# nacho-pancho/binary-image-compression

Hardware: AMD Instinct MI355X
Metric: encode MPixels/s (and MB/s out) at 1/2/4/8 GPUs; bit-exact vs CPU (higher is better)
Workload: dtype u64; 1 GPU; c3: 16384x16384 8-bit gray -> 8 bitplanes -> med -> per-row runs -> Golomb + EG streams per plane (bitplanes formed in registers, not returned: planes NULL) -- the count pass writes the EG stream, the Golomb emission reads the residual rows from it; rows=16384, cols=16384, planes_per_gpu=8, parallelism=dp1 (independent images per GPU)

## Files before the change

### binary-image-compression_amd/csrc/bic_capi.cpp

```cpp
#include "bic_ctx.h"

#include <cctype>
#include <cmath>
#include <map>
#include <new>

#ifdef BIC_STAMPS
namespace bic {
int read_stamps(uint64_t* host, size_t n);
int read_match_stamps(uint64_t* host, size_t n);
}
#endif

namespace {

int ctx_init(bic_ctx* ctx) {
  if (hipStreamCreateWithFlags(&ctx->own, hipStreamNonBlocking) != hipSuccess) return BIC_EDEVICE;
  ctx->cur = ctx->own;
  uint64_t host_lut[bic::kLutWords];
  bic::build_byte_lut(host_lut);
  bic::egad_build_nib(host_lut + bic::kLutEgadNib);
  bic::egad_build_dec_nib(host_lut + bic::kLutEgadDec);
  if (hipMalloc(&ctx->lut, sizeof(host_lut)) != hipSuccess ||
      hipMemcpy(ctx->lut, host_lut, sizeof(host_lut), hipMemcpyHostToDevice) != hipSuccess)
// ... 219 lines not shown
    if (!pnm_int(bytes, n, i, h)) return BIC_EINVAL;
    pnm_skip_comments(bytes, n, i);
    if (!pnm_int(bytes, n, i, mv)) return BIC_EINVAL;
    if (w <= 0 || h <= 0 || mv <= 0 || mv > 65535) return BIC_EINVAL;
    ++i;
  } else {
    return BIC_EINVAL;
  }
  if (i > n) return BIC_EINVAL;
  info->type = type;
  info->cols = (size_t)w;
  info->rows = (size_t)h;
  info->maxval = (int)mv;
  info->data_offset = i;
  return BIC_OK;
}

double bic_enum_codelength(unsigned n, unsigned r) {
  if (r == 0 || r >= n) return 0.0;
  const unsigned m = r * 2 > n ? n - r : r;
  if (m == 1) {
    if ((n & (n - 1)) == 0) {
      unsigned e = 0;
      while ((1u << e) < n) ++e;
      return (double)e;
    }
    return (double)std::log2((long double)n);
  }
  const long double ln = std::lgamma((long double)n + 1.0L) - std::lgamma((long double)m + 1.0L) -
                         std::lgamma((long double)(n - m) + 1.0L);
  return (double)(ln * 1.442695040888963407359924681001892137L);
}

int bic_tile_lentab(unsigned W, uint64_t* lentab) {
  if (W < 1 || W > 64 || !lentab) return BIC_EINVAL;
  const unsigned M = W * W;
  for (unsigned w = 0; w <= M; ++w)
    lentab[w] = (uint64_t)(2.0 + bic_enum_codelength(M, w));
  return BIC_OK;
}

int bic_prof_enable(bic_ctx* ctx, int on) {
  if (!ctx) return BIC_EINVAL;
  ctx->prof_on = on != 0;
  return BIC_OK;
}

int bic_prof_only(bic_ctx* ctx, const char* name) {
  if (!ctx) return BIC_EINVAL;
  ctx->prof_only = name ? name : "";
  return BIC_OK;
}

int bic_prof_collect(bic_ctx* ctx, char* buf, size_t cap) {
  int rc = bind(ctx);
  if (rc) return rc;
  if (!buf || cap == 0) return BIC_EINVAL;
  BIC_HIP(hipStreamSynchronize(ctx->cur));
  std::map<std::string, std::pair<unsigned long, double>> agg;
  for (auto& r : ctx->recs) {
    float ms = 0.f;
    if (hipEventElapsedTime(&ms, r.a, r.b) != hipSuccess) ms = -1.f;
    auto& e = agg[r.name];
    e.first += 1;
    e.second += ms;
    ctx->pool.push_back(r.a);
    ctx->pool.push_back(r.b);
  }
  ctx->recs.clear();
  (void)hipGetLastError();
  std::string outs;
  for (auto& kv : agg) {
    char line[160];
    std::snprintf(line, sizeof line, "%s %lu %.6f\n", kv.first.c_str(), kv.second.first, kv.second.second);
    outs += line;
  }
  std::snprintf(buf, cap, "%s", outs.c_str());
  return outs.size() < cap ? BIC_OK : BIC_ENOSPC;
}

#ifdef BIC_STAMPS
int bic_debug_stamps(uint64_t* host, size_t n) { return bic::read_stamps(host, n); }
int bic_debug_match_stamps(uint64_t* host, size_t n) { return bic::read_match_stamps(host, n); }
#endif

}
```

### binary-image-compression_amd/csrc/bic_kernels.hip

```cpp
#include "bic_device.h"
#include "bic_k1pi.h"
#include "bic_kstat.h"

namespace bic {

__device__ __forceinline__ uint64_t transpose8x8(uint64_t x) {
  uint64_t t;
  t = (x ^ (x >> 7)) & 0x00AA00AA00AA00AAull;
  x = x ^ t ^ (t << 7);
  t = (x ^ (x >> 14)) & 0x0000CCCC0000CCCCull;
  x = x ^ t ^ (t << 14);
  t = (x ^ (x >> 28)) & 0x00000000F0F0F0F0ull;
  x = x ^ t ^ (t << 28);
  return x;
}

template <bool VEC>
__global__ __launch_bounds__(kBlock) void k_bitplanes_u8(const uint8_t* __restrict__ gray, size_t pitch,
                                                         uint32_t rows, uint32_t cols, uint32_t used,
                                                         int plane0, int nplanes, uint64_t* __restrict__ planes,
                                                         uint32_t wpr) {
  const uint32_t groups = (used + 63) / 64;
  const uint64_t gw = (uint64_t)blockIdx.x * kWaves + wave_id();
  if (gw >= (uint64_t)rows * groups) return;
// ... 427 lines not shown
    LaneK k;
    uint64_t D[LW], R[LW];
#pragma unroll
    for (int i = 0; i < LW; ++i) D[i] = PREDICT ? cur[i] ^ up[i] : cur[i];
    const uint64_t dl = wave_shr1_u64(D[LW - 1]);
#pragma unroll
    for (int i = 0; i < LW; ++i) {
      const uint32_t w = w0 + i;
      R[i] = D[i];
      if constexpr (PREDICT) {
        R[i] = D[i] ^ ((D[i] >> 1) | ((i ? D[i - 1] : dl) << 63));
        if (row == 0 && w == 0) R[i] &= ~BIC_MSB;
      }
      R[i] = w < g.used ? (w == g.used - 1 ? R[i] & g.trail : R[i]) : 0;
      lanek_word(k, R[i], (int32_t)(w * 64));
      up[i] = cur[i];
    }
    const uint64_t id = (uint64_t)plane * g.rows + row;
    lanek_store(k, krec + id, kpos + id, sones + id);
    uint64_t* orow = out + (uint64_t)row * g.wpr;
#pragma unroll
    for (int i = 0; i < LW; i += 2)
      if (w0 + i < g.wpr)
        *reinterpret_cast<ulonglong2*>(orow + w0 + i) =
            store_r ? make_ulonglong2(R[i], R[i + 1]) : make_ulonglong2(cur[i], cur[i + 1]);
    for (uint32_t w = 64 * LW + 2 * lane; w < g.wpr; w += 128)
      *reinterpret_cast<ulonglong2*>(orow + w) = make_ulonglong2(0, 0);
#pragma unroll
    for (int i = 0; i < LW; ++i) cur[i] = nxt[i];
  }
}

void launch_pbm_rows(hipStream_t s, const uint8_t* raster, uint64_t stride, const Geom& g, int predict, uint64_t* dst,
                     bool store_resid, uint32_t* sones, int4* krec, uint32_t* kpos, uint32_t* zero) {
  constexpr int RPW = 8;
  const uint32_t wpp = (g.rows + RPW - 1) / RPW;
  const uint32_t grid = (uint32_t)(((uint64_t)wpp * g.nplanes + kWaves - 1) / kWaves);
  const int sr = store_resid && predict ? 1 : 0;
#define BIC_PKS(LW, P) k_pbm_kstat<LW, RPW, P><<<grid, kBlock, 0, s>>>(g, raster, stride, dst, sr, sones, krec, kpos, zero)
  if (g.used <= 128) { if (predict) BIC_PKS(2, true); else BIC_PKS(2, false); }
  else { if (predict) BIC_PKS(4, true); else BIC_PKS(4, false); }
#undef BIC_PKS
}

#ifndef BIC_GRAY_ROWS
#define BIC_GRAY_ROWS 4
#endif
#ifndef BIC_GRAY_ROWS_BM
#define BIC_GRAY_ROWS_BM 1
#endif
constexpr int kGrayRowsP = BIC_GRAY_ROWS, kGrayRowsBM = BIC_GRAY_ROWS_BM;
uint32_t gray_strips(const Geom& g) { return (g.used + 63) / 64; }

__device__ __forceinline__ void perm_t4(uint32_t w0, uint32_t w1, uint32_t w2, uint32_t w3, uint32_t (&out)[4]) {
  const uint32_t a01 = __builtin_amdgcn_perm(w0, w1, 0x04000501u), b01 = __builtin_amdgcn_perm(w0, w1, 0x06020703u);
  const uint32_t a23 = __builtin_amdgcn_perm(w2, w3, 0x04000501u), b23 = __builtin_amdgcn_perm(w2, w3, 0x06020703u);
  out[0] = __builtin_amdgcn_perm(a01, a23, 0x07060302u);
  out[1] = __builtin_amdgcn_perm(a01, a23, 0x05040100u);
  out[2] = __builtin_amdgcn_perm(b01, b23, 0x07060302u);
  out[3] = __builtin_amdgcn_perm(b01, b23, 0x05040100u);
}

__device__ __forceinline__ uint64_t transpose8x8_bs(uint32_t x0, uint32_t x1) {
  uint32_t hi = __builtin_bswap32(x0), lo = __builtin_bswap32(x1);
  uint32_t t;
  t = __builtin_amdgcn_bitop3_b32(lo, lo >> 7, 0x00AA00AAu, 0x28);
  lo = __builtin_amdgcn_bitop3_b32(lo, t, t << 7, 0x96);
  t = __builtin_amdgcn_bitop3_b32(hi, hi >> 7, 0x00AA00AAu, 0x28);
  hi = __builtin_amdgcn_bitop3_b32(hi, t, t << 7, 0x96);
  t = __builtin_amdgcn_bitop3_b32(lo, lo >> 14, 0x0000CCCCu, 0x28);
  lo = __builtin_amdgcn_bitop3_b32(lo, t, t << 14, 0x96);
  t = __builtin_amdgcn_bitop3_b32(hi, hi >> 14, 0x0000CCCCu, 0x28);
  hi = __builtin_amdgcn_bitop3_b32(hi, t, t << 14, 0x96);
  t = __builtin_amdgcn_bitop3_b32(lo, hi << 4, 0xF0F0F0F0u, 0x28);
  lo ^= t;
  hi ^= t >> 4;
  return ((uint64_t)hi << 32) | lo;
}

template <bool FULL = false>
__device__ __forceinline__ void gray_to_planes(const uint4 (&v)[4], uint64_t (&pw)[8], uint64_t mask) {
  uint64_t T[8];
#pragma unroll
  for (int i = 0; i < 4; ++i) {
    T[2 * i] = transpose8x8_bs(v[i].x, v[i].y);
    T[2 * i + 1] = transpose8x8_bs(v[i].z, v[i].w);
  }
  uint32_t XL[4], YL[4], XH[4], YH[4];
  perm_t4((uint32_t)T[0], (uint32_t)T[1], (uint32_t)T[2], (uint32_t)T[3], XL);
  perm_t4((uint32_t)T[4], (uint32_t)T[5], (uint32_t)T[6], (uint32_t)T[7], YL);
  perm_t4((uint32_t)(T[0] >> 32), (uint32_t)(T[1] >> 32), (uint32_t)(T[2] >> 32), (uint32_t)(T[3] >> 32), XH);
  perm_t4((uint32_t)(T[4] >> 32), (uint32_t)(T[5] >> 32), (uint32_t)(T[6] >> 32), (uint32_t)(T[7] >> 32), YH);
#pragma unroll
  for (int b = 0; b < 4; ++b) {
    pw[b] = ((uint64_t)XL[b] << 32) | YL[b];
    pw[4 + b] = ((uint64_t)XH[b] << 32) | YH[b];
    if constexpr (!FULL) {
      pw[b] &= mask;
      pw[4 + b] &= mask;
    }
  }
}

#ifndef BIC_GRAY_PREFETCH
#define BIC_GRAY_PREFETCH 1
#endif
constexpr bool kGrayPrefetch = BIC_GRAY_PREFETCH != 0;
#ifndef BIC_GRAY_BYTEMED
#define BIC_GRAY_BYTEMED 1
#endif
constexpr bool kGrayByteMed = BIC_GRAY_BYTEMED != 0;
template <bool PREDICT, bool STORE_R>
constexpr int gray_rows_per_wave() { return kGrayByteMed && PREDICT && STORE_R ? kGrayRowsBM : kGrayRowsP; }
__device__ __forceinline__ void load64_mis(const uint8_t* src, uint4 (&v)[4]) {
  const uintptr_t a = reinterpret_cast<uintptr_t>(src);
  const uint32_t mis = (uint32_t)(a & 15), bs = mis & 3, dq = mis >> 2;
  const uint4* b = reinterpret_cast<const uint4*>(src - mis);
  uint32_t in[20];
#pragma unroll
  for (int q = 0; q < 4; ++q) {
    const uint4 x = b[q];
    in[4 * q] = x.x;
    in[4 * q + 1] = x.y;
    in[4 * q + 2] = x.z;
    in[4 * q + 3] = x.w;
  }
  const uint4 x4 = mis ? b[4] : make_uint4(0, 0, 0, 0);
  in[16] = x4.x;
  in[17] = x4.y;
  in[18] = x4.z;
  in[19] = x4.w;
#define BIC_MIS_CASE(DQ)                                                                                    \
  case DQ:                                                                                                  \
    _Pragma("unroll") for (int q = 0; q < 4; ++q) v[q] =                                                    \
        make_uint4(__builtin_amdgcn_alignbyte(in[4 * q + DQ + 1], in[4 * q + DQ], bs),                     \
                   __builtin_amdgcn_alignbyte(in[4 * q + DQ + 2], in[4 * q + DQ + 1], bs),                 \
                   __builtin_amdgcn_alignbyte(in[4 * q + DQ + 3], in[4 * q + DQ + 2], bs),                 \
                   __builtin_amdgcn_alignbyte(in[4 * q + DQ + 4], in[4 * q + DQ + 3], bs));                \
    break;
  switch (dq) {
    BIC_MIS_CASE(0)
    BIC_MIS_CASE(1)
    BIC_MIS_CASE(2)
    default: BIC_MIS_CASE(3)
  }
#undef BIC_MIS_CASE
}

struct Raw16 {
  uint4 cur[8], up[8];
};

template <bool PREDICT, bool FULL, bool STORE_R, bool NP8, bool EGS, bool MIS = false, int S16 = 0>
// ... 1420 lines not shown
```

### binary-image-compression_amd/csrc/bic_kstat.h

```cpp
#pragma once
#include "bic_device.h"

namespace bic {

constexpr int32_t kNoOnes = 1 << 30;
constexpr uint32_t kMaxStrips = 4;

__device__ __forceinline__ uint32_t parity_changes(uint64_t x) {
  constexpr uint64_t kEven = 0xAAAAAAAAAAAAAAAAull;
  const uint64_t E = x & kEven, O = x & ~kEven;
  const uint64_t pe = (~x + (E << 1)) & x, po = (~x + (O << 1)) & x;
  return (uint32_t)__popcll(pe & O) + (uint32_t)__popcll(po & E);
}

struct LaneK {
  uint32_t ones = 0, chg = 0;
  int32_t q0 = -kNoOnes, qh = -kNoOnes, ql = kNoOnes, first = -1, last = -1;
};
__device__ __forceinline__ void lanek_word(LaneK& k, uint64_t x, int32_t c0) {
  if (!x) return;
  const int32_t m = __popcll(x), o = (int32_t)k.ones;
  const int32_t pl = c0 + 63 - __builtin_ctzll(x), pf = c0 + __builtin_clzll(x);
  k.q0 = max(k.q0, pl - m - 2 * o);
  k.qh = max(k.qh, pl - m - 3 * o - 1);
  k.ql = min(k.ql, pf - 2 * o - m);
  k.chg += parity_changes(x) + (k.last >= 0 ? (uint32_t)((k.last ^ pf) & 1) : 0u);
  if (k.first < 0) k.first = pf;
  k.last = pl;
  k.ones += m;
}

__device__ __forceinline__ void lanek_store(const LaneK& k, int4* rec, uint32_t* pos, uint32_t* sones) {
  if (__ballot(k.ones != 0) == ~0ull) {
    const int32_t before = dpp_or<0x138>(-1, k.last);
    const uint32_t chg = k.chg + (before >= 0 ? (uint32_t)((before ^ k.first) & 1) : 0u);
    const uint32_t inc = wave_incl_sum_u32(k.ones | (chg << 16));
    const int32_t base = (int32_t)((inc & 0xffffu) - k.ones);
    const int32_t q0 = wave_max(k.q0 - 2 * base);
    const int32_t qh = wave_max(k.qh - 3 * base);
    const int32_t ql = wave_min(k.ql - 2 * base);
    const uint32_t t = lane63_u32(inc), tot = t & 0xffffu;
    const uint32_t f = (uint32_t)__builtin_amdgcn_readlane(k.first, 0);
    const uint32_t last = lane63_u32((uint32_t)k.last);
    if (lane_id() == 0) {
      *rec = make_int4(q0, qh, ql, (int32_t)(tot | (t >> 16 << 16)));
      *pos = (f & 0xffffu) | (last << 16);
      *sones = tot;
    }
    return;
  }
  const uint32_t inc = wave_incl_sum_u32(k.ones);
  const int32_t base = (int32_t)(inc - k.ones);
  const int mx = wave_incl_max(k.last);
  const int32_t before = dpp_or<0x138>(-1, mx);
  uint32_t chg = k.chg;
  int32_t first = -1;
  if (k.ones) {
    if (before >= 0) chg += (uint32_t)((before ^ k.first) & 1);
    else first = k.first;
  }
  const int32_t q0 = wave_max(k.ones ? k.q0 - 2 * base : -kNoOnes);
  const int32_t qh = wave_max(k.ones ? k.qh - 3 * base : -kNoOnes);
  const int32_t ql = wave_min(k.ones ? k.ql - 2 * base : kNoOnes);
  const uint32_t c = wave_sum_u32(chg);
  const int32_t f = wave_max(first);
  const uint32_t tot = lane63_u32(inc);
  const uint32_t last = lane63_u32((uint32_t)mx);
  if (lane_id() == 0) {
    *rec = make_int4(q0, qh, ql, (int32_t)(tot | (c << 16)));
    *pos = ((uint32_t)f & 0xffffu) | (last << 16);
    *sones = tot;
  }
}

__device__ __forceinline__ void strip_word_put(uint32_t* t, int b, uint64_t x, int32_t c0) {
  const int lane = lane_id();
  const uint32_t m = (uint32_t)__popcll(x) | (parity_changes(x) << 8);
  uint32_t hh, hl, lh, ll;
  const uint32_t xh = (uint32_t)(x >> 32), xl = (uint32_t)x;
  asm volatile("v_ffbh_u32 %0, %1" : "=v"(hh) : "v"(xh));
  asm volatile("v_ffbh_u32 %0, %1" : "=v"(hl) : "v"(xl));
  asm volatile("v_ffbl_b32 %0, %1" : "=v"(lh) : "v"(xh));
  asm volatile("v_ffbl_b32 %0, %1" : "=v"(ll) : "v"(xl));
  const uint32_t lz = min(hh, hl + 32u), tz = min(ll, lh + 32u);
  const uint32_t c = ((uint32_t)c0 + lz) | (((uint32_t)c0 + 63u - tz) << 16);
  const uint32_t idx = ((uint32_t)(lane & 7) >> 2) * 256 + 32 * b + 4 * (lane >> 3) + (lane & 3);
  t[idx] = m;
  t[512 + idx] = c;
}
template <int CTRL>
__device__ __forceinline__ int dpp_same(int v) {
  return __builtin_amdgcn_mov_dpp(v, CTRL, 0xf, 0xf, true);
}
__device__ __forceinline__ void strip_records(const uint32_t* t, int np, int4* krec, uint32_t* kpos, uint32_t* sones,
                                              uint64_t id0, uint64_t pstride) {
  const int L = lane_id(), p = L >> 3, j = L & 7;
  const uint4 a0 = *reinterpret_cast<const uint4*>(t + 4 * L);
  const uint4 a1 = *reinterpret_cast<const uint4*>(t + 256 + 4 * L);
  const uint4 c0 = *reinterpret_cast<const uint4*>(t + 512 + 4 * L);
  const uint4 c1 = *reinterpret_cast<const uint4*>(t + 768 + 4 * L);
  const uint32_t av[8] = {a0.x, a0.y, a0.z, a0.w, a1.x, a1.y, a1.z, a1.w};
  const uint32_t cv[8] = {c0.x, c0.y, c0.z, c0.w, c1.x, c1.y, c1.z, c1.w};
  uint32_t ones = 0, chg = 0;
  int32_t first = -1, last = -1, q0 = -kNoOnes, qh = -kNoOnes, ql = kNoOnes;
#pragma unroll
  for (int i = 0; i < 8; ++i) {
    const int32_t m = (int32_t)(av[i] & 0xffu);
    if (m) {
      const int32_t pf = (int32_t)(cv[i] & 0xffffu), pl = (int32_t)(cv[i] >> 16), o = (int32_t)ones;
      chg += (av[i] >> 8) + (last >= 0 ? (uint32_t)((last ^ pf) & 1) : 0u);
      q0 = max(q0, pl - m - 2 * o);
      qh = max(qh, pl - m - 1 - 3 * o);
      ql = min(ql, pf - m - 2 * o);
      if (first < 0) first = pf;
      last = pl;
      ones += (uint32_t)m;
    }
  }
  uint32_t inc = ones;
  int32_t lmax = last;
#pragma unroll
  for (int d = 1; d < 8; d <<= 1) {
    const uint32_t o = d == 1 ? (uint32_t)dpp_or<0x111>(0, (int)inc) : d == 2 ? (uint32_t)dpp_or<0x112>(0, (int)inc)
                                                                             : (uint32_t)dpp_or<0x114>(0, (int)inc);
    const int32_t lm = d == 1 ? dpp_or<0x111>(-1, lmax) : d == 2 ? dpp_or<0x112>(-1, lmax) : dpp_or<0x114>(-1, lmax);
    if (j >= d) {
      inc += o;
      lmax = max(lmax, lm);
    }
  }
  const int32_t lprev = dpp_or<0x111>(-1, lmax);
  const int32_t before = j ? lprev : -1;
  const int32_t B = (int32_t)(inc - ones);
  if (ones) {
    if (before >= 0) chg += (uint32_t)((before ^ first) & 1);
    q0 -= 2 * B;
    qh -= 3 * B;
    ql -= 2 * B;
  }
  int32_t f = ones ? first : INT_MAX;
  uint32_t tot = ones;
#define BIC_RED8(CTRL)                          \
  q0 = max(q0, dpp_same<CTRL>(q0));             \
  qh = max(qh, dpp_same<CTRL>(qh));             \
  ql = min(ql, dpp_same<CTRL>(ql));             \
  f = min(f, dpp_same<CTRL>(f));                \
  last = max(last, dpp_same<CTRL>(last));       \
  chg += (uint32_t)dpp_same<CTRL>((int)chg);    \
  tot += (uint32_t)dpp_same<CTRL>((int)tot);
  BIC_RED8(0xB1)
  BIC_RED8(0x4E)
  BIC_RED8(0x141)
#undef BIC_RED8
  if (j == 0 && p < np) {
    const uint64_t id = id0 + (uint64_t)p * pstride;
    krec[id] = make_int4(q0, qh, ql, (int32_t)(tot | (chg << 16)));
    kpos[id] = ((uint32_t)(f == INT_MAX ? -1 : f) & 0xffffu) | ((uint32_t)last << 16);
    sones[id] = tot;
  }
}

struct RowK {
  int32_t q0, qh, ql;
  uint32_t ones, chg;
};
struct RowKRaw {
  int4 v[kMaxStrips];
  uint32_t pp[kMaxStrips];
};
__device__ __forceinline__ RowKRaw row_kstats_load(const int4* rec, const uint32_t* pos, uint32_t ns) {
  RowKRaw q;
#pragma unroll
  for (uint32_t s = 0; s < kMaxStrips; ++s) {
    q.v[s] = s < ns ? rec[s] : make_int4(0, 0, 0, 0);
    q.pp[s] = s < ns ? pos[s] : 0u;
  }
  return q;
}
__device__ __forceinline__ RowK row_kstats_combine(const RowKRaw& q, uint32_t cols) {
  const int4* v = q.v;
  const uint32_t* pp = q.pp;
  RowK r{0, 0, 0, 0, 0};
  int32_t last = -1;
#pragma unroll
  for (uint32_t s = 0; s < kMaxStrips; ++s) {
    const uint32_t o = (uint32_t)v[s].w & 0xffffu;
    if (!o) continue;
    r.q0 = max(r.q0, v[s].x - 2 * (int32_t)r.ones);
    r.qh = max(r.qh, v[s].y - 3 * (int32_t)r.ones);
    r.ql = min(r.ql, v[s].z - 2 * (int32_t)r.ones);
    r.chg += ((uint32_t)v[s].w >> 16) + (uint32_t)((last ^ (int32_t)(int16_t)(pp[s] & 0xffffu)) & 1);
    r.ones += o;
    last = (int16_t)(pp[s] >> 16);
  }
  r.chg += (uint32_t)((last ^ (int32_t)cols) & 1);
  return r;
}
__device__ __forceinline__ RowK row_kstats(const int4* rec, const uint32_t* pos, uint32_t ns, uint32_t cols) {
  return row_kstats_combine(row_kstats_load(rec, pos, ns), cols);
}

}
```

### binary-image-compression_amd/pybic/__init__.py

```python
import ctypes as C
import os

import numpy as np

PKG = os.path.dirname(os.path.dirname(os.path.abspath(__file__)))
LIB_PATH = os.environ.get("BIC_LIB_PATH") or os.path.join(PKG, "lib", "libbic.so")

BIC_OK, BIC_EINVAL, BIC_ENOMEM, BIC_EDEVICE, BIC_ENOSPC, BIC_ENODEV, BIC_EDATA = range(7)
CODER_GOLOMB, CODER_EG, CODER_EG_ADAPTIVE = 0, 1, 2

EXPORTS = [
    "bic_ctx_create", "bic_ctx_destroy", "bic_ctx_set_stream", "bic_ctx_get_stream", "bic_ctx_own_stream",
    "bic_sync",
    "bic_strerror", "bic_device_count", "bic_reserve", "bic_bitplanes_u8", "bic_med_residual",
    "bic_encode_planes", "bic_encode_planes2", "bic_ctx_set_option", "bic_encode_slot_words", "bic_golomb_encode_samples", "bic_patch_encode",
    "bic_pack_streams", "bic_prof_enable", "bic_prof_collect", "bic_prof_only", "bic_enum_codelength", "bic_tile_lentab",
    "bic_malloc", "bic_free", "bic_memcpy_h2d", "bic_memcpy_d2h", "bic_memset", "bic_pbm_unpack", "bic_pbm_pack",
    "bic_patch_search", "bic_match_encode", "bic_set_match_parts", "bic_encode_gray",
    "bic_bitplanes_u8_range", "bic_encode_gray_range", "bic_encode_planes_packed", "bic_encode_gray_packed",
    "bic_row_index", "bic_decode_planes", "bic_pgm_bitplanes", "bic_pnm_parse_header",
    "bic_gf2_transpose", "bic_gf2_mul", "bic_planes_to_gray", "bic_match_encode_inv", "bic_match_encode_var", "bic_egad_row_index",
    "bic_encode_gray16", "bic_encode_gray16_packed", "bic_bitplanes_u16", "bic_decode_gray",
    "bic_encode_pbm", "bic_encode_pbm_packed", "bic_decode_pbm",
    "bic_bsvd_update_coefficients", "bic_bsvd_update_dictionary", "bic_bsvd_learn",
]

GF2_AB, GF2_ATB, GF2_ABT, GF2_ATBT = 0, 1, 2, 3


class PnmInfo(C.Structure):
    _fields_ = [("type", C.c_int), ("rows", C.c_size_t), ("cols", C.c_size_t), ("maxval", C.c_int),
                ("data_offset", C.c_size_t)]


class BicError(RuntimeError):
    def __init__(self, code, what=""):
        self.code = code
        super().__init__(f"{what}: bic error {code} ({_strerror(code)})")


_lib = None


def _strerror(code):
    try:
        return load().bic_strerror(code).decode()
    except Exception:
        return "?"


def load(path=LIB_PATH):
    global _lib
    if _lib is not None:
        return _lib
    if not os.path.exists(path):
        raise OSError(f"{path} not built; run make -C binary-image-compression_amd")
    L = C.CDLL(path)
    vp, sz, u64, i32, u32 = C.c_void_p, C.c_size_t, C.c_uint64, C.c_int, C.c_uint

    def sig(name, res, args):
        f = getattr(L, name)
        f.restype, f.argtypes = res, args

    sig("bic_ctx_create", i32, [i32, C.POINTER(vp)])
    sig("bic_ctx_destroy", i32, [vp])
    sig("bic_ctx_set_stream", i32, [vp, vp])
    sig("bic_ctx_get_stream", vp, [vp])
    sig("bic_ctx_own_stream", vp, [vp])
    sig("bic_sync", i32, [vp])
    sig("bic_strerror", C.c_char_p, [i32])
    sig("bic_device_count", i32, [C.POINTER(i32)])
    sig("bic_reserve", i32, [vp, i32, sz, sz])
    sig("bic_bitplanes_u8", i32, [vp, vp, sz, sz, sz, i32, vp, sz])
    sig("bic_med_residual", i32, [vp, vp, i32, sz, sz, sz, i32, vp, vp])
    sig("bic_encode_planes", i32, [vp, vp, i32, sz, sz, sz, i32, i32, vp, sz, vp])
    sig("bic_encode_slot_words", sz, [sz, sz, i32])
    sig("bic_encode_planes2", i32, [vp, vp, i32, sz, sz, sz, i32, vp, sz, vp, vp, sz, vp])
    sig("bic_ctx_set_option", i32, [vp, i32, C.c_long])
    sig("bic_golomb_encode_samples", i32, [vp, vp, sz, u64, u64, u32, vp, sz, vp])
    sig("bic_patch_encode", i32, [vp, vp, sz, sz, sz, u32, vp, vp, vp, vp, vp, vp, vp, sz, vp])
    sig("bic_pack_streams", i32, [vp, vp, i32, sz, vp, vp, vp])
    sig("bic_prof_enable", i32, [vp, i32])
    sig("bic_prof_collect", i32, [vp, C.c_char_p, sz])
    sig("bic_prof_only", i32, [vp, C.c_char_p])
    sig("bic_enum_codelength", C.c_double, [u32, u32])
    sig("bic_tile_lentab", i32, [u32, vp])
    sig("bic_malloc", i32, [vp, sz, C.POINTER(vp)])
    sig("bic_free", i32, [vp, vp])
    sig("bic_memcpy_h2d", i32, [vp, vp, vp, sz])
    sig("bic_memcpy_d2h", i32, [vp, vp, vp, sz])
    sig("bic_memset", i32, [vp, vp, i32, sz])
    sig("bic_pbm_unpack", i32, [vp, vp, sz, sz, vp, sz])
    sig("bic_pbm_pack", i32, [vp, vp, sz, sz, sz, vp])
    sig("bic_patch_search", i32, [vp, vp, sz, sz, sz, u32, vp, vp, vp])
    sig("bic_match_encode", i32, [vp, vp, sz, sz, sz, u32, u32, u32, vp, vp, vp, vp, vp, vp, vp, vp, vp, sz, vp])
    sig("bic_set_match_parts", i32, [vp, u32])
    sig("bic_match_encode_inv", i32, [vp, vp, sz, sz, sz, u32, u32, u32, vp, vp, vp, vp, vp, vp, vp, vp, vp, vp, sz, vp])
    sig("bic_egad_row_index", i32, [vp, vp, i32, sz, sz, sz, i32, vp])
    sig("bic_match_encode_var", i32, [vp, i32, vp, sz, sz, sz, u32, u32, u32, vp, vp, vp, vp, vp, vp, vp, vp, vp, sz, vp])
    sig("bic_encode_gray", i32, [vp, vp, sz, sz, sz, i32, vp, sz, i32, vp, sz, vp, vp, sz, vp])
    sig("bic_bitplanes_u8_range", i32, [vp, vp, sz, sz, sz, i32, i32, vp, sz])
    sig("bic_encode_gray_range", i32, [vp, vp, sz, sz, sz, i32, i32, vp, sz, i32, vp, sz, vp, vp, sz, vp])
    sig("bic_encode_planes_packed", i32, [vp, vp, i32, sz, sz, sz, i32, vp, sz, vp, vp, vp, sz, vp, vp, vp])
    sig("bic_encode_gray_packed", i32, [vp, vp, sz, sz, sz, i32, i32, vp, sz, i32, vp, sz, vp, vp, vp, sz, vp, vp, vp])
    sig("bic_row_index", i32, [vp, vp, i32, sz, sz, sz, i32, vp])
    sig("bic_decode_planes", i32, [vp, i32, vp, sz, vp, vp, vp, i32, sz, sz, sz, i32, vp, vp])
    sig("bic_pgm_bitplanes", i32, [vp, vp, sz, sz, i32, i32, i32, vp, sz])
    sig("bic_pnm_parse_header", i32, [C.c_char_p, sz, C.POINTER(PnmInfo)])
    sig("bic_gf2_transpose", i32, [vp, vp, sz, sz, sz, vp, sz])
    sig("bic_gf2_mul", i32, [vp, i32, vp, sz, sz, sz, vp, sz, sz, sz, vp, sz, sz, sz])
    sig("bic_planes_to_gray", i32, [vp, vp, i32, i32, sz, sz, sz, i32, vp, sz])
    sig("bic_bitplanes_u16", i32, [vp, vp, sz, sz, sz, i32, i32, i32, vp, sz])
    sig("bic_encode_gray16", i32, [vp, vp, sz, sz, sz, i32, i32, i32, vp, sz, i32, vp, sz, vp, vp, sz, vp])
    sig("bic_encode_gray16_packed", i32, [vp, vp, sz, sz, sz, i32, i32, i32, vp, sz, i32, vp, sz, vp, vp, vp, sz, vp,
                                          vp, vp])
    sig("bic_decode_gray", i32, [vp, i32, vp, sz, vp, vp, vp, i32, i32, sz, sz, i32, vp, i32, i32, vp, sz])
    sig("bic_encode_pbm", i32, [vp, vp, sz, i32, sz, sz, vp, sz, i32, vp, sz, vp, vp, sz, vp])
    sig("bic_encode_pbm_packed", i32, [vp, vp, sz, i32, sz, sz, vp, sz, i32, vp, sz, vp, vp, vp, sz, vp, vp, vp])
    sig("bic_decode_pbm", i32, [vp, i32, vp, sz, vp, vp, vp, i32, sz, sz, i32, vp, vp, sz])
    sig("bic_bsvd_update_coefficients", i32, [vp, vp, sz, sz, sz, vp, sz, sz, vp, sz, vp])
    sig("bic_bsvd_update_dictionary", i32, [vp, vp, sz, sz, sz, vp, sz, sz, vp, sz, vp])
    sig("bic_bsvd_learn", i32, [vp, vp, sz, vp, sz, sz, sz, vp, sz, sz, vp, sz, sz, C.POINTER(sz)])
    _lib = L
    return L


def as_u64(t):
    return t.detach().cpu().numpy().view(np.uint64)


def stream_bytes(words_i64, nbits):
    nw = (int(nbits) + 63) // 64
    return as_u64(words_i64[:nw]).tobytes()


def _p(t):
    return None if t is None else C.c_void_p(t.data_ptr())
# ... 7 lines not shown
        self.torch = torch
        self.lib = load()
        self.device = device
        h = C.c_void_p()
        rc = self.lib.bic_ctx_create(device, C.byref(h))
        if rc != BIC_OK:
            raise BicError(rc, f"bic_ctx_create({device})")
        self.h = h
        self.dev = torch.device("cuda", device)

    def close(self):
        if getattr(self, "h", None):
            self.lib.bic_ctx_destroy(self.h)
            self.h = None

    def __del__(self):
        try:
            self.close()
        except Exception:
            pass

    def _bind_stream(self):
        s = self.torch.cuda.current_stream(self.dev).cuda_stream
        self.lib.bic_ctx_set_stream(self.h, C.c_void_p(s) if s else None)

    def _chk(self, rc, what):
        if rc != BIC_OK:
            raise BicError(rc, what)

    def sync(self):
        rc = self.lib.bic_sync(self.h)
        self._chk(rc, "bic_sync")

    def empty_i64(self, *shape):
        return self.torch.empty(*shape, dtype=self.torch.int64, device=self.dev)

    def to_dev(self, a):
        a = np.ascontiguousarray(a)
        if a.dtype == np.uint64:
            a = a.view(np.int64)
        elif a.dtype == np.uint32:
            a = a.view(np.int32)
        return self.torch.from_numpy(a).to(self.dev)

    def reserve(self, nplanes, rows, cols):
        self._chk(self.lib.bic_reserve(self.h, nplanes, rows, cols), "bic_reserve")

    def prof_enable(self, on=True):
        self._chk(self.lib.bic_prof_enable(self.h, int(on)), "bic_prof_enable")

    def prof_only(self, name=None):
        self._chk(self.lib.bic_prof_only(self.h, name.encode() if name else None), "bic_prof_only")

    def prof_collect(self):
        buf = C.create_string_buffer(1 << 16)
        self._chk(self.lib.bic_prof_collect(self.h, buf, len(buf)), "bic_prof_collect")
        out = {}
        for line in buf.value.decode().splitlines():
            name, n, ms = line.split()
            out[name] = (int(n), float(ms))
        return out

    def bitplanes_u8(self, gray, cols=None, nplanes=8, wpr=None, out=None, plane0=0):
        rows, pitch = gray.shape
        cols = pitch if cols is None else cols
        wpr = wpr or (cols + 63) // 64
        if out is None:
            out = self.empty_i64(nplanes, rows, wpr)
        self._bind_stream()
        if plane0:
            self._chk(self.lib.bic_bitplanes_u8_range(self.h, _p(gray), pitch, rows, cols, plane0, nplanes, _p(out),
                                                      wpr), "bic_bitplanes_u8_range")
        else:
            self._chk(self.lib.bic_bitplanes_u8(self.h, _p(gray), pitch, rows, cols, nplanes, _p(out), wpr),
                      "bic_bitplanes_u8")
        return out

    def med_residual(self, planes, cols, predict=True, want_resid=True, want_weight=True):
        planes = planes if planes.dim() == 3 else planes.unsqueeze(0)
        n, rows, wpr = planes.shape
        resid = self.empty_i64(n, rows, wpr) if want_resid else None
        w = self.torch.zeros(n, dtype=self.torch.int64, device=self.dev) if want_weight else None
        self._bind_stream()
        self._chk(self.lib.bic_med_residual(self.h, _p(planes), n, rows, cols, wpr, int(predict),
                                            _p(resid), _p(w)), "bic_med_residual")
        return resid, w

    def slot_words(self, rows, cols, coder):
        return int(self.lib.bic_encode_slot_words(rows, cols, coder))

    def encode_planes(self, planes, cols, predict=True, coder=CODER_GOLOMB, slot_words=None,
                      out=None, plane_bits=None):
        planes = planes if planes.dim() == 3 else planes.unsqueeze(0)
        n, rows, wpr = planes.shape
        slot_words = slot_words or self.slot_words(rows, cols, coder)
        if out is None:
            out = self.empty_i64(n, slot_words)
        if plane_bits is None:
            plane_bits = self.empty_i64(n)
        self._bind_stream()
        self._chk(self.lib.bic_encode_planes(self.h, _p(planes), n, rows, cols, wpr, int(predict), coder,
                                             _p(out), slot_words, _p(plane_bits)), "bic_encode_planes")
        return out, plane_bits

    def encode_planes2(self, planes, cols, predict=True, golomb=True, eg=True, slots=(None, None),
                       outs=(None, None), bits=(None, None)):
# ... 464 lines not shown
```

### include/bic.h

```cpp
#ifndef BIC_H
#define BIC_H

#include <stddef.h>
#include <stdint.h>

#ifdef __cplusplus
extern "C" {
#endif

#define BIC_OK 0
#define BIC_EINVAL 1
#define BIC_ENOMEM 2
#define BIC_EDEVICE 3
#define BIC_ENOSPC 4
#define BIC_ENODEV 5
#define BIC_EDATA 6

#define BIC_CODER_GOLOMB 0
#define BIC_CODER_EG 1
#define BIC_CODER_EG_ADAPTIVE 2

typedef struct bic_ctx bic_ctx;

int bic_ctx_create(int device, bic_ctx** out);
// ... 97 lines not shown
                     uint32_t* bestd, uint32_t* weights, uint8_t* modes, uint64_t* resid,
                     uint64_t* stream_match, uint64_t* stream_nomatch, size_t cap_words, uint64_t* stats);
int bic_match_encode_inv(bic_ctx* ctx, const uint64_t* plane, size_t rows, size_t cols, size_t wpr, unsigned W,
                         unsigned T, unsigned R, const double* enuml, uint32_t* besti, uint32_t* bestj,
                         uint32_t* bestd, uint32_t* weights, uint8_t* modes, uint8_t* inverted, uint64_t* resid,
                         uint64_t* stream_match, uint64_t* stream_nomatch, size_t cap_words, uint64_t* stats);
int bic_match_encode_var(bic_ctx* ctx, int variant, const uint64_t* plane, size_t rows, size_t cols, size_t wpr,
                         unsigned W, unsigned T, unsigned R, const double* enuml, uint32_t* besti, uint32_t* bestj,
                         uint32_t* bestd, uint32_t* weights, uint8_t* modes, uint64_t* resid, uint64_t* stream_match,
                         uint64_t* stream_nomatch, size_t cap_words, uint64_t* stats);
int bic_set_match_parts(bic_ctx* ctx, unsigned parts);

double bic_enum_codelength(unsigned n, unsigned r);
int bic_tile_lentab(unsigned W, uint64_t* lentab);

int bic_pack_streams(bic_ctx* ctx, const uint64_t* slots, int nplanes, size_t slot_words,
                     const uint64_t* plane_bits, uint64_t* dst, uint64_t* word_off);

int bic_pbm_unpack(bic_ctx* ctx, const uint8_t* raster, size_t rows, size_t cols, uint64_t* plane, size_t wpr);
int bic_pbm_pack(bic_ctx* ctx, const uint64_t* plane, size_t rows, size_t cols, size_t wpr, uint8_t* raster);

typedef struct {
  int type;
  size_t rows, cols;
  int maxval;
  size_t data_offset;
} bic_pnm_info;
int bic_pnm_parse_header(const uint8_t* bytes, size_t n, bic_pnm_info* info);
int bic_pgm_bitplanes(bic_ctx* ctx, const uint8_t* raster, size_t rows, size_t cols, int maxval, int plane0,
                      int nplanes, uint64_t* planes, size_t wpr);
int bic_planes_to_gray(bic_ctx* ctx, const uint64_t* planes, int plane0, int nplanes, size_t rows, size_t cols,
                       size_t wpr, int sample_bytes, void* gray, size_t pitch);

#define BIC_GF2_AB 0
#define BIC_GF2_ATB 1
#define BIC_GF2_ABT 2
#define BIC_GF2_ATBT 3
int bic_gf2_transpose(bic_ctx* ctx, const uint64_t* src, size_t rows, size_t cols, size_t wpr, uint64_t* dst,
                      size_t dst_wpr);
int bic_gf2_mul(bic_ctx* ctx, int op, const uint64_t* A, size_t a_rows, size_t a_cols, size_t a_wpr,
                const uint64_t* B, size_t b_rows, size_t b_cols, size_t b_wpr, uint64_t* C, size_t c_rows,
                size_t c_cols, size_t c_wpr);

int bic_bsvd_update_coefficients(bic_ctx* ctx, uint64_t* E, size_t n, size_t m, size_t e_wpr, const uint64_t* D,
                                 size_t p, size_t d_wpr, uint64_t* A, size_t a_wpr, uint64_t* changed);
int bic_bsvd_update_dictionary(bic_ctx* ctx, uint64_t* E, size_t n, size_t m, size_t e_wpr, uint64_t* D, size_t p,
                               size_t d_wpr, const uint64_t* A, size_t a_wpr, uint64_t* changed);
int bic_bsvd_learn(bic_ctx* ctx, const uint64_t* X, size_t x_wpr, uint64_t* E, size_t n, size_t m, size_t e_wpr,
                   uint64_t* D, size_t p, size_t d_wpr, uint64_t* A, size_t a_wpr, size_t max_iter, size_t* iters);

int bic_prof_enable(bic_ctx* ctx, int on);
int bic_prof_collect(bic_ctx* ctx, char* buf, size_t cap);
int bic_prof_only(bic_ctx* ctx, const char* name);

#ifdef __cplusplus
}
#endif
#endif
```

Measured before the change: 7.277 million MPix/s.

## Rework gray-to-bitplane transpose and strip stats with packed 16-bit arithmetic

Replaces the 8x8 bit-transpose-plus-byte-permute path in gray_to_planes with a byte permute followed by a three-stage bitop3 butterfly. Moves the strip word statistics into a new shared header that packs q0/ql and first/last into 16-bit halves. This cuts the per-lane state and the number of DPP reductions in the kstat kernel, and it makes parity_changes cheaper. The aim is fewer ALU instructions and fewer registers in the per-plane statistics pass. The 16-bit packing depends on sentinel offsets to stay in range. A profiling entry point that reads row-class counters is also added.

```diff
diff --git a/binary-image-compression_amd/csrc/bic_capi.cpp b/binary-image-compression_amd/csrc/bic_capi.cpp
--- a/binary-image-compression_amd/csrc/bic_capi.cpp
+++ b/binary-image-compression_amd/csrc/bic_capi.cpp
@@ -295,6 +295,17 @@
   return BIC_OK;
 }
 
+int bic_prof_row_classes(bic_ctx* ctx, uint32_t counts[4]) {
+  int rc = bind(ctx);
+  if (rc) return rc;
+  if (!counts || !ctx->scratch) return BIC_EINVAL;
+  BIC_HIP(hipStreamSynchronize(ctx->cur));
+  uint32_t c[6];
+  BIC_HIP(hipMemcpy(c, ctx->scratch, sizeof c, hipMemcpyDeviceToHost));
+  counts[0] = c[2], counts[1] = c[3], counts[2] = c[4], counts[3] = c[5];
+  return BIC_OK;
+}
+
 int bic_prof_collect(bic_ctx* ctx, char* buf, size_t cap) {
   int rc = bind(ctx);
   if (rc) return rc;
diff --git a/binary-image-compression_amd/csrc/bic_kernels.hip b/binary-image-compression_amd/csrc/bic_kernels.hip
--- a/binary-image-compression_amd/csrc/bic_kernels.hip
+++ b/binary-image-compression_amd/csrc/bic_kernels.hip
@@ -503,53 +503,14 @@
 constexpr int kGrayRowsP = BIC_GRAY_ROWS, kGrayRowsBM = BIC_GRAY_ROWS_BM;
 uint32_t gray_strips(const Geom& g) { return (g.used + 63) / 64; }
 
-__device__ __forceinline__ void perm_t4(uint32_t w0, uint32_t w1, uint32_t w2, uint32_t w3, uint32_t (&out)[4]) {
-  const uint32_t a01 = __builtin_amdgcn_perm(w0, w1, 0x04000501u), b01 = __builtin_amdgcn_perm(w0, w1, 0x06020703u);
-  const uint32_t a23 = __builtin_amdgcn_perm(w2, w3, 0x04000501u), b23 = __builtin_amdgcn_perm(w2, w3, 0x06020703u);
-  out[0] = __builtin_amdgcn_perm(a01, a23, 0x07060302u);
-  out[1] = __builtin_amdgcn_perm(a01, a23, 0x05040100u);
-  out[2] = __builtin_amdgcn_perm(b01, b23, 0x07060302u);
-  out[3] = __builtin_amdgcn_perm(b01, b23, 0x05040100u);
-}
-
-__device__ __forceinline__ uint64_t transpose8x8_bs(uint32_t x0, uint32_t x1) {
-  uint32_t hi = __builtin_bswap32(x0), lo = __builtin_bswap32(x1);
-  uint32_t t;
-  t = __builtin_amdgcn_bitop3_b32(lo, lo >> 7, 0x00AA00AAu, 0x28);
-  lo = __builtin_amdgcn_bitop3_b32(lo, t, t << 7, 0x96);
-  t = __builtin_amdgcn_bitop3_b32(hi, hi >> 7, 0x00AA00AAu, 0x28);
-  hi = __builtin_amdgcn_bitop3_b32(hi, t, t << 7, 0x96);
-  t = __builtin_amdgcn_bitop3_b32(lo, lo >> 14, 0x0000CCCCu, 0x28);
-  lo = __builtin_amdgcn_bitop3_b32(lo, t, t << 14, 0x96);
-  t = __builtin_amdgcn_bitop3_b32(hi, hi >> 14, 0x0000CCCCu, 0x28);
-  hi = __builtin_amdgcn_bitop3_b32(hi, t, t << 14, 0x96);
-  t = __builtin_amdgcn_bitop3_b32(lo, hi << 4, 0xF0F0F0F0u, 0x28);
-  lo ^= t;
-  hi ^= t >> 4;
-  return ((uint64_t)hi << 32) | lo;
-}
-
 template <bool FULL = false>
 __device__ __forceinline__ void gray_to_planes(const uint4 (&v)[4], uint64_t (&pw)[8], uint64_t mask) {
-  uint64_t T[8];
-#pragma unroll
-  for (int i = 0; i < 4; ++i) {
-    T[2 * i] = transpose8x8_bs(v[i].x, v[i].y);
-    T[2 * i + 1] = transpose8x8_bs(v[i].z, v[i].w);
-  }
-  uint32_t XL[4], YL[4], XH[4], YH[4];
-  perm_t4((uint32_t)T[0], (uint32_t)T[1], (uint32_t)T[2], (uint32_t)T[3], XL);
-  perm_t4((uint32_t)T[4], (uint32_t)T[5], (uint32_t)T[6], (uint32_t)T[7], YL);
-  perm_t4((uint32_t)(T[0] >> 32), (uint32_t)(T[1] >> 32), (uint32_t)(T[2] >> 32), (uint32_t)(T[3] >> 32), XH);
-  perm_t4((uint32_t)(T[4] >> 32), (uint32_t)(T[5] >> 32), (uint32_t)(T[6] >> 32), (uint32_t)(T[7] >> 32), YH);
-#pragma unroll
-  for (int b = 0; b < 4; ++b) {
-    pw[b] = ((uint64_t)XL[b] << 32) | YL[b];
-    pw[4 + b] = ((uint64_t)XH[b] << 32) | YH[b];
-    if constexpr (!FULL) {
-      pw[b] &= mask;
-      pw[4 + b] &= mask;
-    }
+  const uint32_t d[16] = {v[0].x, v[0].y, v[0].z, v[0].w, v[1].x, v[1].y, v[1].z, v[1].w,
+                          v[2].x, v[2].y, v[2].z, v[2].w, v[3].x, v[3].y, v[3].z, v[3].w};
+  gray64_to_planes(d, pw);
+  if constexpr (!FULL) {
+#pragma unroll
+    for (int b = 0; b < 8; ++b) pw[b] &= mask;
   }
 }
 
diff --git a/binary-image-compression_amd/csrc/bic_kstat.h b/binary-image-compression_amd/csrc/bic_kstat.h
--- a/binary-image-compression_amd/csrc/bic_kstat.h
+++ b/binary-image-compression_amd/csrc/bic_kstat.h
@@ -1,17 +1,11 @@
 #pragma once
 #include "bic_device.h"
+#include "bic_strip.h"
 
 namespace bic {
 
 constexpr int32_t kNoOnes = 1 << 30;
 constexpr uint32_t kMaxStrips = 4;
-
-__device__ __forceinline__ uint32_t parity_changes(uint64_t x) {
-  constexpr uint64_t kEven = 0xAAAAAAAAAAAAAAAAull;
-  const uint64_t E = x & kEven, O = x & ~kEven;
-  const uint64_t pe = (~x + (E << 1)) & x, po = (~x + (O << 1)) & x;
-  return (uint32_t)__popcll(pe & O) + (uint32_t)__popcll(po & E);
-}
 
 struct LaneK {
   uint32_t ones = 0, chg = 0;
@@ -75,15 +69,8 @@
 
 __device__ __forceinline__ void strip_word_put(uint32_t* t, int b, uint64_t x, int32_t c0) {
   const int lane = lane_id();
-  const uint32_t m = (uint32_t)__popcll(x) | (parity_changes(x) << 8);
-  uint32_t hh, hl, lh, ll;
-  const uint32_t xh = (uint32_t)(x >> 32), xl = (uint32_t)x;
-  asm volatile("v_ffbh_u32 %0, %1" : "=v"(hh) : "v"(xh));
-  asm volatile("v_ffbh_u32 %0, %1" : "=v"(hl) : "v"(xl));
-  asm volatile("v_ffbl_b32 %0, %1" : "=v"(lh) : "v"(xh));
-  asm volatile("v_ffbl_b32 %0, %1" : "=v"(ll) : "v"(xl));
-  const uint32_t lz = min(hh, hl + 32u), tz = min(ll, lh + 32u);
-  const uint32_t c = ((uint32_t)c0 + lz) | (((uint32_t)c0 + 63u - tz) << 16);
+  uint32_t m, c;
+  strip_word_entry(x, c0, m, c);
   const uint32_t idx = ((uint32_t)(lane & 7) >> 2) * 256 + 32 * b + 4 * (lane >> 3) + (lane & 3);
   t[idx] = m;
   t[512 + idx] = c;
@@ -101,24 +88,10 @@
   const uint4 c1 = *reinterpret_cast<const uint4*>(t + 768 + 4 * L);
   const uint32_t av[8] = {a0.x, a0.y, a0.z, a0.w, a1.x, a1.y, a1.z, a1.w};
   const uint32_t cv[8] = {c0.x, c0.y, c0.z, c0.w, c1.x, c1.y, c1.z, c1.w};
-  uint32_t ones = 0, chg = 0;
-  int32_t first = -1, last = -1, q0 = -kNoOnes, qh = -kNoOnes, ql = kNoOnes;
-#pragma unroll
-  for (int i = 0; i < 8; ++i) {
-    const int32_t m = (int32_t)(av[i] & 0xffu);
-    if (m) {
-      const int32_t pf = (int32_t)(cv[i] & 0xffffu), pl = (int32_t)(cv[i] >> 16), o = (int32_t)ones;
-      chg += (av[i] >> 8) + (last >= 0 ? (uint32_t)((last ^ pf) & 1) : 0u);
-      q0 = max(q0, pl - m - 2 * o);
-      qh = max(qh, pl - m - 1 - 3 * o);
-      ql = min(ql, pf - m - 2 * o);
-      if (first < 0) first = pf;
-      last = pl;
-      ones += (uint32_t)m;
-    }
-  }
+  const StripPart sp = strip_part(av, cv);
+  const uint32_t ones = sp.ones;
   uint32_t inc = ones;
-  int32_t lmax = last;
+  int32_t lmax = pk_hi(sp.f);
 #pragma unroll
   for (int d = 1; d < 8; d <<= 1) {
     const uint32_t o = d == 1 ? (uint32_t)dpp_or<0x111>(0, (int)inc) : d == 2 ? (uint32_t)dpp_or<0x112>(0, (int)inc)
@@ -131,32 +104,26 @@
   }
   const int32_t lprev = dpp_or<0x111>(-1, lmax);
   const int32_t before = j ? lprev : -1;
-  const int32_t B = (int32_t)(inc - ones);
-  if (ones) {
-    if (before >= 0) chg += (uint32_t)((before ^ first) & 1);
-    q0 -= 2 * B;
-    qh -= 3 * B;
-    ql -= 2 * B;
-  }
-  int32_t f = ones ? first : INT_MAX;
-  uint32_t tot = ones;
-#define BIC_RED8(CTRL)                          \
-  q0 = max(q0, dpp_same<CTRL>(q0));             \
-  qh = max(qh, dpp_same<CTRL>(qh));             \
-  ql = min(ql, dpp_same<CTRL>(ql));             \
-  f = min(f, dpp_same<CTRL>(f));                \
-  last = max(last, dpp_same<CTRL>(last));       \
-  chg += (uint32_t)dpp_same<CTRL>((int)chg);    \
-  tot += (uint32_t)dpp_same<CTRL>((int)tot);
+  uint32_t q, ct, f = sp.f;
+  int32_t qh;
+  strip_part_rebase(sp, inc - ones, before, q, qh, ct);
+#define BIC_RED8(CTRL)                                     \
+  q = pk_max16(q, (uint32_t)dpp_same<CTRL>((int)q));       \
+  f = pk_max16(f, (uint32_t)dpp_same<CTRL>((int)f));       \
+  qh = max(qh, dpp_same<CTRL>(qh));                        \
+  ct += (uint32_t)dpp_same<CTRL>((int)ct);
   BIC_RED8(0xB1)
   BIC_RED8(0x4E)
   BIC_RED8(0x141)
 #undef BIC_RED8
   if (j == 0 && p < np) {
     const uint64_t id = id0 + (uint64_t)p * pstride;
-    krec[id] = make_int4(q0, qh, ql, (int32_t)(tot | (chg << 16)));
-    kpos[id] = ((uint32_t)(f == INT_MAX ? -1 : f) & 0xffffu) | ((uint32_t)last << 16);
-    sones[id] = tot;
+    int32_t rec[4];
+    uint32_t pos;
+    strip_record(q, f, qh, ct, rec, pos);
+    krec[id] = make_int4(rec[0], rec[1], rec[2], rec[3]);
+    kpos[id] = pos;
+    sones[id] = ct & 0xffffu;
   }
 }
 
diff --git a/binary-image-compression_amd/csrc/bic_strip.h b/binary-image-compression_amd/csrc/bic_strip.h
--- /dev/null
+++ b/binary-image-compression_amd/csrc/bic_strip.h
@@ -0,0 +1,174 @@
+#pragma once
+#include "bic_k1pi.h"
+
+namespace bic {
+
+BIC_HDI uint32_t perm_b32(uint32_t s0, uint32_t s1, uint32_t sel) {
+#if defined(__HIP_DEVICE_COMPILE__)
+  return __builtin_amdgcn_perm(s0, s1, sel);
+#else
+  const uint64_t v = ((uint64_t)s0 << 32) | s1;
+  uint32_t r = 0;
+  for (int i = 0; i < 4; ++i) r |= (uint32_t)((v >> (8 * ((sel >> (8 * i)) & 7u))) & 0xffu) << (8 * i);
+  return r;
+#endif
+}
+template <int TT>
+BIC_HDI uint32_t bitop3(uint32_t a, uint32_t b, uint32_t c) {
+#if defined(__HIP_DEVICE_COMPILE__)
+  return __builtin_amdgcn_bitop3_b32(a, b, c, TT);
+#else
+  uint32_t r = 0;
+  for (int i = 0; i < 8; ++i)
+    if ((TT >> i) & 1) r |= (i & 4 ? a : ~a) & (i & 2 ? b : ~b) & (i & 1 ? c : ~c);
+  return r;
+#endif
+}
+BIC_HDI uint32_t pk_add16(uint32_t a, uint32_t b) {
+#if defined(__HIP_DEVICE_COMPILE__)
+  typedef short s2 __attribute__((ext_vector_type(2)));
+  return __builtin_bit_cast(uint32_t, (s2)(__builtin_bit_cast(s2, a) + __builtin_bit_cast(s2, b)));
+#else
+  return ((a + b) & 0xffffu) | ((a & 0xffff0000u) + (b & 0xffff0000u));
+#endif
+}
+BIC_HDI uint32_t pk_max16(uint32_t a, uint32_t b) {
+#if defined(__HIP_DEVICE_COMPILE__)
+  typedef short s2 __attribute__((ext_vector_type(2)));
+  return __builtin_bit_cast(uint32_t, __builtin_elementwise_max(__builtin_bit_cast(s2, a), __builtin_bit_cast(s2, b)));
+#else
+  const int16_t al = (int16_t)a, bl = (int16_t)b, ah = (int16_t)(a >> 16), bh = (int16_t)(b >> 16);
+  return (uint32_t)(uint16_t)(al > bl ? al : bl) | ((uint32_t)(uint16_t)(ah > bh ? ah : bh) << 16);
+#endif
+}
+BIC_HDI uint32_t nonzero01(uint32_t v) {
+#if defined(__HIP_DEVICE_COMPILE__)
+  uint32_t r;
+  asm("v_min_u32 %0, 1, %1" : "=v"(r) : "v"(v));
+  return r;
+#else
+  return v ? 1u : 0u;
+#endif
+}
+BIC_HDI int32_t pk_hi(uint32_t a) { return (int32_t)a >> 16; }
+BIC_HDI int32_t pk_lo(uint32_t a) { return (int32_t)(int16_t)(a & 0xffffu); }
+BIC_HDI uint32_t pk_negpos(uint32_t v, int scale = 1) {
+#if defined(__HIP_DEVICE_COMPILE__)
+  return (uint32_t)__mul24((int)v, scale * -65535);
+#else
+  return v * (uint32_t)(scale * -65535);
+#endif
+}
+
+BIC_HDI void perm_t4(uint32_t w0, uint32_t w1, uint32_t w2, uint32_t w3, uint32_t (&out)[4]) {
+  const uint32_t a01 = perm_b32(w0, w1, 0x04000501u), b01 = perm_b32(w0, w1, 0x06020703u);
+  const uint32_t a23 = perm_b32(w2, w3, 0x04000501u), b23 = perm_b32(w2, w3, 0x06020703u);
+  out[0] = perm_b32(a01, a23, 0x07060302u);
+  out[1] = perm_b32(a01, a23, 0x05040100u);
+  out[2] = perm_b32(b01, b23, 0x07060302u);
+  out[3] = perm_b32(b01, b23, 0x05040100u);
+}
+
+BIC_HDI void gray32_to_planes(const uint32_t* d, uint32_t (&half)[8]) {
+  uint32_t r[8], t[4];
+  perm_t4(d[0], d[2], d[4], d[6], t);
+BIC_UNROLL
+  for (int i = 0; i < 4; ++i) r[i] = t[i];
+  perm_t4(d[1], d[3], d[5], d[7], t);
+BIC_UNROLL
+  for (int i = 0; i < 4; ++i) r[4 + i] = t[i];
+#define BIC_BFLY(S, M)                                                  \
+  BIC_UNROLL                                                            \
+  for (int i = 0; i < 8; ++i)                                           \
+    if (!(i & S)) {                                                     \
+      const uint32_t a = r[i], b = r[i + S];                            \
+      r[i] = bitop3<0xE4>(a, b >> S, M);      \
+      r[i + S] = bitop3<0xE4>(a << S, b, M);  \
+    }
+  BIC_BFLY(4, 0xF0F0F0F0u)
+  BIC_BFLY(2, 0xCCCCCCCCu)
+  BIC_BFLY(1, 0xAAAAAAAAu)
+#undef BIC_BFLY
+BIC_UNROLL
+  for (int b = 0; b < 8; ++b) half[b] = r[7 - b];
+}
+BIC_HDI void gray64_to_planes(const uint32_t (&d)[16], uint64_t (&pw)[8]) {
+  uint32_t h[8], l[8];
+  gray32_to_planes(d, h);
+  gray32_to_planes(d + 8, l);
+BIC_UNROLL
+  for (int b = 0; b < 8; ++b) pw[b] = ((uint64_t)h[b] << 32) | l[b];
+}
+
+BIC_HDI uint32_t parity_changes(uint64_t x) {
+  constexpr uint64_t kEven = 0xAAAAAAAAAAAAAAAAull;
+  const uint64_t pe = (~x + ((x & kEven) << 1)) & x, y = x & (x - 1);
+  const uint32_t hi = bitop3<0x78>((uint32_t)(pe >> 32), (uint32_t)(y >> 32), 0xAAAAAAAAu);
+  const uint32_t lo = bitop3<0x78>((uint32_t)pe, (uint32_t)y, 0xAAAAAAAAu);
+#if defined(__HIP_DEVICE_COMPILE__)
+  return (uint32_t)__popc(hi) + (uint32_t)__popc(lo);
+#else
+  return (uint32_t)__builtin_popcount(hi) + (uint32_t)__builtin_popcount(lo);
+#endif
+}
+
+constexpr int kStripNoneHi = -16384, kStripNoneLo = -28000;
+constexpr uint32_t kStripNone = ((uint32_t)(uint16_t)(int16_t)kStripNoneHi << 16) | (uint16_t)(int16_t)kStripNoneLo;
+BIC_HDI void strip_word_entry(uint64_t x, int32_t c0, uint32_t& a, uint32_t& c) {
+#if defined(__HIP_DEVICE_COMPILE__)
+  const uint32_t xh = (uint32_t)(x >> 32), xl = (uint32_t)x;
+  a = (uint32_t)__popcll(x) | (parity_changes(x) << 8);
+  uint32_t hh, hl, lh, ll;
+  asm volatile("v_ffbh_u32 %0, %1" : "=v"(hh) : "v"(xh));
+  asm volatile("v_ffbh_u32 %0, %1" : "=v"(hl) : "v"(xl));
+  asm volatile("v_ffbl_b32 %0, %1" : "=v"(lh) : "v"(xh));
+  asm volatile("v_ffbl_b32 %0, %1" : "=v"(ll) : "v"(xl));
+  const uint32_t lz = min(hh, hl + 32u), tz = min(ll, lh + 32u);
+#else
+  a = (uint32_t)__builtin_popcountll(x) | (parity_changes(x) << 8);
+  const uint32_t lz = x ? (uint32_t)__builtin_clzll(x) : 0u, tz = x ? (uint32_t)__builtin_ctzll(x) : 0u;
+#endif
+  const uint32_t bl = (uint32_t)(c0 + 63 - kStripNoneHi), bf = (uint32_t)(-kStripNoneLo - c0);
+  c = a ? perm_b32(bl - tz, bf - lz, 0x05040100u) : 0u;
+}
+
+struct StripPart {
+  uint32_t ones, chg, q, f;
+  int32_t qh;
+};
+BIC_HDI StripPart strip_part(const uint32_t (&av)[8], const uint32_t (&cv)[8]) {
+  StripPart s{0u, 0u, kStripNone, (uint32_t)(-1 - kStripNoneHi) << 16, -(1 << 30)};
+  uint32_t ones2 = kStripNone, ones3 = (uint32_t)(1 - kStripNoneHi);
+BIC_UNROLL
+  for (int i = 0; i < 8; ++i) {
+    const uint32_t m = av[i] & 0xffu, c = cv[i], nz = nonzero01(m);
+    s.chg += (av[i] >> 8) + bitop3<0x28>(s.f >> 16, c, nz);
+    s.q = pk_max16(s.q, pk_add16(pk_add16(c, pk_negpos(m)), ones2));
+    const int32_t t = (int32_t)(c >> 16) - (int32_t)m - (int32_t)ones3;
+    s.qh = s.qh > t ? s.qh : t;
+    s.f = pk_max16(s.f, c);
+    ones2 += pk_negpos(m, 2);
+    ones3 += 3 * m;
+    s.ones += m;
+  }
+  s.f = pk_add16(s.f, kStripNone);
+  return s;
+}
+BIC_HDI void strip_part_rebase(const StripPart& s, uint32_t B, int32_t before, uint32_t& q, int32_t& qh, uint32_t& ct) {
+  const uint32_t nz = nonzero01(s.ones), pb = (uint32_t)(before + 1);
+  const uint32_t link = bitop3<0x28>((uint32_t)before, s.f, pb < nz ? pb : nz) - bitop3<0x28>(~0u, s.f, nz);
+  q = pk_add16(s.q, pk_negpos(B, 2));
+  qh = s.qh - 3 * (int32_t)B;
+  ct = s.ones | ((s.chg + link) << 16);
+}
+BIC_HDI void strip_record(uint32_t q, uint32_t f, int32_t qh, uint32_t ct, int32_t (&rec)[4], uint32_t& pos) {
+  constexpr int32_t kNone = 1 << 30;
+  const bool any = (ct & 0xffffu) != 0;
+  rec[0] = any ? pk_hi(q) : -kNone;
+  rec[1] = any ? qh : -kNone;
+  rec[2] = any ? -pk_lo(q) : kNone;
+  rec[3] = (int32_t)ct;
+  pos = any ? ((uint32_t)(-pk_lo(f)) & 0xffffu) | ((uint32_t)pk_hi(f) << 16) : ~0u;
+}
+
+}
diff --git a/binary-image-compression_amd/pybic/__init__.py b/binary-image-compression_amd/pybic/__init__.py
--- a/binary-image-compression_amd/pybic/__init__.py
+++ b/binary-image-compression_amd/pybic/__init__.py
@@ -23,6 +23,7 @@
     "bic_encode_gray16", "bic_encode_gray16_packed", "bic_bitplanes_u16", "bic_decode_gray",
     "bic_encode_pbm", "bic_encode_pbm_packed", "bic_decode_pbm",
     "bic_bsvd_update_coefficients", "bic_bsvd_update_dictionary", "bic_bsvd_learn",
+    "bic_prof_row_classes",
 ]
 
 GF2_AB, GF2_ATB, GF2_ABT, GF2_ATBT = 0, 1, 2, 3
@@ -83,6 +84,7 @@
     sig("bic_prof_enable", i32, [vp, i32])
     sig("bic_prof_collect", i32, [vp, C.c_char_p, sz])
     sig("bic_prof_only", i32, [vp, C.c_char_p])
+    sig("bic_prof_row_classes", i32, [vp, C.POINTER(C.c_uint32)])
     sig("bic_enum_codelength", C.c_double, [u32, u32])
     sig("bic_tile_lentab", i32, [u32, vp])
     sig("bic_malloc", i32, [vp, sz, C.POINTER(vp)])
@@ -196,6 +198,11 @@
     def prof_only(self, name=None):
         self._chk(self.lib.bic_prof_only(self.h, name.encode() if name else None), "bic_prof_only")
 
+    def row_classes(self):
+        c = (C.c_uint32 * 4)()
+        self._chk(self.lib.bic_prof_row_classes(self.h, c), "bic_prof_row_classes")
+        return tuple(int(x) for x in c)
+
     def prof_collect(self):
         buf = C.create_string_buffer(1 << 16)
         self._chk(self.lib.bic_prof_collect(self.h, buf, len(buf)), "bic_prof_collect")
diff --git a/include/bic.h b/include/bic.h
--- a/include/bic.h
+++ b/include/bic.h
@@ -173,6 +173,7 @@
 int bic_prof_enable(bic_ctx* ctx, int on);
 int bic_prof_collect(bic_ctx* ctx, char* buf, size_t cap);
 int bic_prof_only(bic_ctx* ctx, const char* name);
+int bic_prof_row_classes(bic_ctx* ctx, uint32_t counts[4]);
 
 #ifdef __cplusplus
 }
```

Result: slower. 7.109 million MPix/s (-2.3%).
